# zhenfeizhang/falcon-r1cs

Hardware: AMD Instinct MI355X
Metric: falcon1024_verify_with_ntt_r1cs_witnesses_per_sec (higher is better)
Workload: dtype u32; 1 GPU; falcon-1024 full verify-with-ntt witness (NTT ladder + mod_q + pointwise + l2-norm), batch=65536 signatures per GPU per step (BASELINE configs[2] on every GPU); logn=10, batch_per_gpu=65536, chunk=32768, encoding=bls12-381-fr montgomery (arkworks witness_assignment bytes), seed=0x46414c434f4e31, signatures_failing_range_checks=0, ranks_seen=1, hbm_plan_bytes=166888865792, hbm_plan_limit_bytes=259200000000

## Files before the change

### falcon-r1cs_amd/csrc/frw_keccak.h

```cpp
#pragma once
#include <hip/hip_runtime.h>
#include <stdint.h>

namespace frw {

static __constant__ uint64_t KECCAK_RC[24] = {
    0x0000000000000001ull, 0x0000000000008082ull, 0x800000000000808aull, 0x8000000080008000ull, 0x000000000000808bull,
    0x0000000080000001ull, 0x8000000080008081ull, 0x8000000000008009ull, 0x000000000000008aull, 0x0000000000000088ull,
    0x0000000080008009ull, 0x000000008000000aull, 0x000000008000808bull, 0x800000000000008bull, 0x8000000000008089ull,
    0x8000000000008003ull, 0x8000000000008002ull, 0x8000000000000080ull, 0x000000000000800aull, 0x800000008000000aull,
    0x8000000080008081ull, 0x8000000000008080ull, 0x0000000080000001ull, 0x8000000080008008ull};

__device__ __forceinline__ uint64_t rol64(uint64_t x, int n) { return (x << n) | (x >> (64 - n)); }

__device__ __forceinline__ void keccak_f1600(uint64_t (&a)[25])
{
#pragma unroll 1
    for (int r = 0; r < 24; r++) {
        uint64_t c0 = a[0] ^ a[5] ^ a[10] ^ a[15] ^ a[20];
        uint64_t c1 = a[1] ^ a[6] ^ a[11] ^ a[16] ^ a[21];
        uint64_t c2 = a[2] ^ a[7] ^ a[12] ^ a[17] ^ a[22];
        uint64_t c3 = a[3] ^ a[8] ^ a[13] ^ a[18] ^ a[23];
        uint64_t c4 = a[4] ^ a[9] ^ a[14] ^ a[19] ^ a[24];
        const uint64_t d0 = c4 ^ rol64(c1, 1), d1 = c0 ^ rol64(c2, 1), d2 = c1 ^ rol64(c3, 1), d3 = c2 ^ rol64(c4, 1),
                       d4 = c3 ^ rol64(c0, 1);
        const uint64_t b0 = a[0] ^ d0;
        const uint64_t b10 = rol64(a[1] ^ d1, 1), b20 = rol64(a[2] ^ d2, 62), b5 = rol64(a[3] ^ d3, 28), b15 = rol64(a[4] ^ d4, 27);
        const uint64_t b16 = rol64(a[5] ^ d0, 36), b1 = rol64(a[6] ^ d1, 44), b11 = rol64(a[7] ^ d2, 6), b21 = rol64(a[8] ^ d3, 55),
                       b6 = rol64(a[9] ^ d4, 20);
        const uint64_t b7 = rol64(a[10] ^ d0, 3), b17 = rol64(a[11] ^ d1, 10), b2 = rol64(a[12] ^ d2, 43), b12 = rol64(a[13] ^ d3, 25),
                       b22 = rol64(a[14] ^ d4, 39);
        const uint64_t b23 = rol64(a[15] ^ d0, 41), b8 = rol64(a[16] ^ d1, 45), b18 = rol64(a[17] ^ d2, 15), b3 = rol64(a[18] ^ d3, 21),
                       b13 = rol64(a[19] ^ d4, 8);
        const uint64_t b14 = rol64(a[20] ^ d0, 18), b24 = rol64(a[21] ^ d1, 2), b9 = rol64(a[22] ^ d2, 61), b19 = rol64(a[23] ^ d3, 56),
                       b4 = rol64(a[24] ^ d4, 14);
        a[0] = b0 ^ (~b1 & b2) ^ KECCAK_RC[r]; a[1] = b1 ^ (~b2 & b3); a[2] = b2 ^ (~b3 & b4); a[3] = b3 ^ (~b4 & b0); a[4] = b4 ^ (~b0 & b1);
        a[5] = b5 ^ (~b6 & b7); a[6] = b6 ^ (~b7 & b8); a[7] = b7 ^ (~b8 & b9); a[8] = b8 ^ (~b9 & b5); a[9] = b9 ^ (~b5 & b6);
        a[10] = b10 ^ (~b11 & b12); a[11] = b11 ^ (~b12 & b13); a[12] = b12 ^ (~b13 & b14); a[13] = b13 ^ (~b14 & b10); a[14] = b14 ^ (~b10 & b11);
        a[15] = b15 ^ (~b16 & b17); a[16] = b16 ^ (~b17 & b18); a[17] = b17 ^ (~b18 & b19); a[18] = b18 ^ (~b19 & b15); a[19] = b19 ^ (~b15 & b16);
        a[20] = b20 ^ (~b21 & b22); a[21] = b21 ^ (~b22 & b23); a[22] = b22 ^ (~b23 & b24); a[23] = b23 ^ (~b24 & b20); a[24] = b24 ^ (~b20 & b21);
    }
}

}
```

### falcon-r1cs_amd/csrc/frw_prepare.hip

```cpp
#include <hip/hip_runtime.h>
#include <stdint.h>
#include "frw_device.h"
#include "frw_keccak.h"

namespace frw {

constexpr int SHAKE256_RATE = 136;
constexpr int NONCE_LEN = 40;

__global__ __launch_bounds__(BLOCK) void hash_to_point_kernel(int logn, size_t batch, const uint8_t *__restrict__ nonces,
                                                              const uint8_t *__restrict__ msgs,
                                                              const uint64_t *__restrict__ msg_off, uint16_t *__restrict__ hm)
{
    const size_t s = (size_t)blockIdx.x * blockDim.x + threadIdx.x;
    if (s >= batch) return;
    const int n = 1 << logn;
    const uint8_t *nonce = nonces + s * NONCE_LEN;
    const uint8_t *msg = msgs + msg_off[s];
    const uint64_t o0 = msg_off[s], o1 = msg_off[s + 1];
    const size_t total = NONCE_LEN + (size_t)(o1 >= o0 ? o1 - o0 : 0);
    uint64_t st[25];
#pragma unroll
    for (int i = 0; i < 25; i++) st[i] = 0;
    for (size_t pos = 0;; pos += SHAKE256_RATE) {
#pragma unroll
        for (int l = 0; l < SHAKE256_RATE / 8; l++) {
            uint64_t w = 0;
#pragma unroll
            for (int b = 0; b < 8; b++) {
                const size_t p = pos + (size_t)(l * 8 + b);
                uint32_t byte = 0;
                if (p < NONCE_LEN) byte = nonce[p];
                else if (p < total) byte = msg[p - NONCE_LEN];
                else if (p == total) byte = 0x1F;
                w |= (uint64_t)byte << (8 * b);
            }
            st[l] ^= w;
        }
        const bool last = total < pos + SHAKE256_RATE;
        if (last) st[16] ^= 0x8000000000000000ull;
        keccak_f1600(st);
        if (last) break;
    }
    uint16_t *out = hm + s * (size_t)n;
    int cnt = 0;
    while (cnt < n) {
#pragma unroll
        for (int w = 0; w < SHAKE256_RATE / 2; w++) {
            const uint64_t lane = st[w / 4];
            const int sh = (w % 4) * 16;
            const uint32_t v = (uint32_t)((lane >> sh) & 0xff) << 8 | (uint32_t)((lane >> (sh + 8)) & 0xff);
            if (v < 5 * Q && cnt < n) out[cnt++] = (uint16_t)(v % Q);
        }
        if (cnt < n) keccak_f1600(st);
    }
}

__global__ __launch_bounds__(BLOCK) void decode_public_keys_kernel(int logn, size_t batch, const uint8_t *__restrict__ pk_bytes,
                                                                   uint16_t *__restrict__ pk, int32_t *__restrict__ status)
{
    const int n = 1 << logn;
    const size_t pk_len = 1 + (size_t)14 * n / 8;
    const size_t idx = (size_t)blockIdx.x * blockDim.x + threadIdx.x;
    if (idx >= batch * (size_t)n) return;
    const size_t s = idx >> logn;
    const int k = (int)(idx & (size_t)(n - 1));
    const uint8_t *p = pk_bytes + s * pk_len;
    const int bit = 14 * k, off = bit & 7;
    const uint8_t *q = p + 1 + (bit >> 3);
    uint32_t acc = (uint32_t)q[0] << 16 | (uint32_t)q[1] << 8;
    if (off + 14 > 16) acc |= q[2];
    const uint32_t c = (acc >> (24 - 14 - off)) & 0x3fffu;
    pk[idx] = (uint16_t)c;
    if (c >= Q || (k == 0 && p[0] != (uint8_t)logn)) atomicMax(&status[s], ST_DECODE);
}

__global__ __launch_bounds__(BLOCK) void decode_signatures_kernel(int logn, size_t batch, const uint8_t *__restrict__ sig_bytes,
                                                                  size_t sig_len, uint16_t *__restrict__ sig,
                                                                  uint8_t *__restrict__ nonce_out, int32_t *__restrict__ status)
{
    const size_t s = (size_t)blockIdx.x * blockDim.x + threadIdx.x;
    if (s >= batch) return;
    const int n = 1 << logn;
    const uint8_t *p = sig_bytes + s * sig_len;
    uint16_t *out = sig + s * (size_t)n;
    bool ok = sig_len > 1 + NONCE_LEN && p[0] == (uint8_t)(0x30 + logn);
    if (ok && nonce_out)
        for (int i = 0; i < NONCE_LEN; i++) nonce_out[s * NONCE_LEN + i] = p[1 + i];
    const uint8_t *body = p + 1 + NONCE_LEN;
    const size_t body_len = ok ? sig_len - 1 - NONCE_LEN : 0;
    size_t v = 0;
    uint32_t acc = 0;
    int acc_len = 0;
    for (int u = 0; ok && u < n; u++) {
        if (v >= body_len) { ok = false; break; }
        acc = (acc << 8) | body[v++];
        const uint32_t b = acc >> acc_len;
        const uint32_t sign = b & 128u;
        uint32_t m = b & 127u;
        for (;;) {
            if (acc_len == 0) {
                if (v >= body_len) { ok = false; break; }
                acc = (acc << 8) | body[v++];
                acc_len = 8;
            }
            acc_len--;
            if ((acc >> acc_len) & 1u) break;
            m += 128;
            if (m > 2047) { ok = false; break; }
        }
        if (sign && m == 0) ok = false;
        if (ok) out[u] = (uint16_t)(sign ? Q - m : m);
    }
    if (ok && (acc & ((1u << acc_len) - 1u))) ok = false;
    for (; ok && v < body_len; v++)
        if (body[v]) ok = false;
    status[s] = ok ? ST_OK : ST_DECODE;
}

hipError_t launch_hash_to_point(int logn, size_t batch, const uint8_t *nonces, const uint8_t *msgs, const uint64_t *msg_off,
                                uint16_t *hm, hipStream_t st)
{
    if (batch == 0) return hipSuccess;
    hipLaunchKernelGGL(hash_to_point_kernel, dim3((unsigned)((batch + BLOCK - 1) / BLOCK)), dim3(BLOCK), 0, st, logn, batch, nonces,
                       msgs, msg_off, hm);
    return hipGetLastError();
}

hipError_t launch_decode_public_keys(int logn, size_t batch, const uint8_t *pk_bytes, uint16_t *pk, int32_t *status, hipStream_t st)
{
    if (batch == 0) return hipSuccess;
    hipError_t e = hipMemsetAsync(status, 0, batch * sizeof(int32_t), st);
    if (e != hipSuccess) return e;
    const size_t total = batch << logn;
    hipLaunchKernelGGL(decode_public_keys_kernel, dim3((unsigned)((total + BLOCK - 1) / BLOCK)), dim3(BLOCK), 0, st, logn, batch,
                       pk_bytes, pk, status);
    return hipGetLastError();
}

hipError_t launch_decode_signatures(int logn, size_t batch, const uint8_t *sig_bytes, size_t sig_len, uint16_t *sig,
                                    uint8_t *nonce_out, int32_t *status, hipStream_t st)
{
    if (batch == 0) return hipSuccess;
    hipLaunchKernelGGL(decode_signatures_kernel, dim3((unsigned)((batch + BLOCK - 1) / BLOCK)), dim3(BLOCK), 0, st, logn, batch,
                       sig_bytes, sig_len, sig, nonce_out, status);
    return hipGetLastError();
}

}
```

Baseline: 1.296 million signatures/s.

## Rewrite input-preparation kernels: paired-lane Keccak, vectorized decoders, batched stores

Hash-to-point now splits each Keccak-f1600 state across two lanes, each holding 32-bit halves and exchanging words through DPP swaps. Absorption uses 8-byte loads and output coefficients are gathered into 16-byte stores. Public-key decode uses one block per key with 8 coefficients per thread and a block-wide OR instead of a memset plus atomics. Signature decode reads 16-byte pieces through an LDS ring and decodes 8 codewords per step with clz. These changes target uncoalesced byte-wise loads and serial scalar work in the preprocessing stage, at the cost of more complex code and the risk of alignment or edge-case bugs.

Result: no change. 1.295 million signatures/s (median of 2 runs) (-0.1%).

```diff
diff --git a/falcon-r1cs_amd/csrc/frw_codec.h b/falcon-r1cs_amd/csrc/frw_codec.h
--- /dev/null
+++ b/falcon-r1cs_amd/csrc/frw_codec.h
@@ -0,0 +1,114 @@
+#pragma once
+#include <hip/hip_runtime.h>
+#include <stddef.h>
+#include <stdint.h>
+
+namespace frw {
+
+constexpr uint32_t CODEC_Q = 12289;
+constexpr int SIG_HEADER_LEN = 1 + 40;
+
+constexpr uint32_t SIG_RING_WORDS = 32;
+
+template <class Fetch, class Ring> struct SigBodyReader {
+    Fetch fetch;
+    Ring ring;
+    uint4 s0, s1;
+    uint32_t ns;
+    uint32_t rd, wr;
+    uint32_t ahead;
+    size_t piece;
+    size_t end_off;
+    size_t left;
+    uint64_t win;
+    int have;
+
+    __host__ __device__ __forceinline__ SigBodyReader(Fetch f, Ring r, unsigned body_misalign, size_t body_len)
+        : fetch(f), ring(r), ns(0), rd(1), wr(16), piece(4), end_off(body_misalign + body_len), left(body_misalign + body_len), win(0), have(0)
+    {
+        s0 = s1 = make_uint4(0, 0, 0, 0);
+        for (uint32_t k = 0; k < 4; k++)
+            if (16 * (size_t)k < end_off) put_piece(4 * k, fetch(k));
+        ahead = ring.get(0);
+        for (unsigned i = 0; i < body_misalign / 4; i++) (void)next_word();
+        win = (uint64_t)next_word() << 32;
+        have = 32 - 8 * (int)(body_misalign & 3);
+        win <<= 8 * (body_misalign & 3);
+    }
+
+    __host__ __device__ __forceinline__ void put_piece(uint32_t at, uint4 p)
+    {
+        ring.put(at % SIG_RING_WORDS, p.x);
+        ring.put((at + 1) % SIG_RING_WORDS, p.y);
+        ring.put((at + 2) % SIG_RING_WORDS, p.z);
+        ring.put((at + 3) % SIG_RING_WORDS, p.w);
+    }
+
+    __host__ __device__ __forceinline__ void boundary()
+    {
+        if (ns >= 1) { put_piece(wr, s0); wr += 4; }
+        if (ns == 2) { put_piece(wr, s1); wr += 4; }
+        const uint32_t avail = wr - rd;
+        ns = avail >= 16 ? 0u : avail >= 12 ? 1u : 2u;
+        if (ns >= 1 && 16 * piece < end_off) s0 = fetch(piece);
+        if (ns == 2 && 16 * (piece + 1) < end_off) s1 = fetch(piece + 1);
+        piece += ns;
+    }
+
+    __host__ __device__ __forceinline__ uint32_t next_word()
+    {
+        uint32_t w = __builtin_bswap32(ahead);
+        ahead = ring.get(rd % SIG_RING_WORDS);
+        rd++;
+        if (left < 4) {
+            w = left ? w & ~(0xffffffffu >> (8 * (unsigned)left)) : 0u;
+            left = 0;
+        } else {
+            left -= 4;
+        }
+        return w;
+    }
+
+    __host__ __device__ __forceinline__ bool codeword(uint32_t &coeff)
+    {
+        if (have <= 32) {
+            win |= (uint64_t)next_word() << (32 - have);
+            have += 32;
+        }
+        const uint32_t top = (uint32_t)(win >> 32);
+        const uint32_t z = (uint32_t)__builtin_clz((top << 8) | 0x8000u);
+        const uint32_t m = ((top >> 24) & 127u) + 128u * z;
+        const bool neg = (top >> 31) != 0;
+        win <<= 9 + z;
+        have -= 9 + (int)z;
+        coeff = neg ? CODEC_Q - m : m;
+        return z <= 15 && !(neg && m == 0);
+    }
+
+    __host__ __device__ __forceinline__ bool rest_is_zero()
+    {
+        uint32_t acc = (uint32_t)(win >> 32) | (uint32_t)win;
+        while (left) {
+            boundary();
+            for (int i = 0; i < 8; i++) acc |= next_word();
+        }
+        return acc == 0;
+    }
+};
+
+template <class Fetch, class Ring, class Store8>
+__host__ __device__ __forceinline__ bool sig_decode_body(Fetch f, Ring ring, unsigned body_misalign, size_t body_len, int n, Store8 store)
+{
+    SigBodyReader<Fetch, Ring> r(f, ring, body_misalign, body_len);
+    bool ok = true;
+    for (int u = 0; ok && u < n; u += 8) {
+        uint32_t c[8];
+        r.boundary();
+#pragma unroll
+        for (int j = 0; j < 8; j++) ok &= r.codeword(c[j]);
+        if (ok) store(u, c);
+    }
+    return ok && r.rest_is_zero();
+}
+
+}
diff --git a/falcon-r1cs_amd/csrc/frw_keccak.h b/falcon-r1cs_amd/csrc/frw_keccak.h
--- a/falcon-r1cs_amd/csrc/frw_keccak.h
+++ b/falcon-r1cs_amd/csrc/frw_keccak.h
@@ -42,4 +42,49 @@
     }
 }
 
+__device__ __forceinline__ uint32_t keccak_pair_swap(uint32_t x)
+{
+    return (uint32_t)__builtin_amdgcn_update_dpp(0, (int)x, 0xB1 , 0xf, 0xf, false);
 }
+
+template <int R> __device__ __forceinline__ uint32_t rol64_half(uint32_t own)
+{
+    static_assert(R >= 0 && R < 64 && R != 32, "a rotation of Keccak-f[1600]");
+    if (R == 0) return own;
+    const uint32_t other = keccak_pair_swap(own);
+    return R < 32 ? __builtin_amdgcn_alignbit(own, other, 32 - R) : __builtin_amdgcn_alignbit(other, own, 64 - R);
+}
+
+__device__ __forceinline__ void keccak_f1600_pair(uint32_t (&a)[25], uint32_t half)
+{
+#pragma unroll 1
+    for (int r = 0; r < 24; r++) {
+        const uint32_t c0 = a[0] ^ a[5] ^ a[10] ^ a[15] ^ a[20];
+        const uint32_t c1 = a[1] ^ a[6] ^ a[11] ^ a[16] ^ a[21];
+        const uint32_t c2 = a[2] ^ a[7] ^ a[12] ^ a[17] ^ a[22];
+        const uint32_t c3 = a[3] ^ a[8] ^ a[13] ^ a[18] ^ a[23];
+        const uint32_t c4 = a[4] ^ a[9] ^ a[14] ^ a[19] ^ a[24];
+        const uint32_t d0 = c4 ^ rol64_half<1>(c1), d1 = c0 ^ rol64_half<1>(c2), d2 = c1 ^ rol64_half<1>(c3), d3 = c2 ^ rol64_half<1>(c4),
+                       d4 = c3 ^ rol64_half<1>(c0);
+        const uint32_t b0 = a[0] ^ d0;
+        const uint32_t b10 = rol64_half<1>(a[1] ^ d1), b20 = rol64_half<62>(a[2] ^ d2), b5 = rol64_half<28>(a[3] ^ d3),
+                       b15 = rol64_half<27>(a[4] ^ d4);
+        const uint32_t b16 = rol64_half<36>(a[5] ^ d0), b1 = rol64_half<44>(a[6] ^ d1), b11 = rol64_half<6>(a[7] ^ d2),
+                       b21 = rol64_half<55>(a[8] ^ d3), b6 = rol64_half<20>(a[9] ^ d4);
+        const uint32_t b7 = rol64_half<3>(a[10] ^ d0), b17 = rol64_half<10>(a[11] ^ d1), b2 = rol64_half<43>(a[12] ^ d2),
+                       b12 = rol64_half<25>(a[13] ^ d3), b22 = rol64_half<39>(a[14] ^ d4);
+        const uint32_t b23 = rol64_half<41>(a[15] ^ d0), b8 = rol64_half<45>(a[16] ^ d1), b18 = rol64_half<15>(a[17] ^ d2),
+                       b3 = rol64_half<21>(a[18] ^ d3), b13 = rol64_half<8>(a[19] ^ d4);
+        const uint32_t b14 = rol64_half<18>(a[20] ^ d0), b24 = rol64_half<2>(a[21] ^ d1), b9 = rol64_half<61>(a[22] ^ d2),
+                       b19 = rol64_half<56>(a[23] ^ d3), b4 = rol64_half<14>(a[24] ^ d4);
+        const uint64_t rc = KECCAK_RC[r];
+        a[0] = b0 ^ (~b1 & b2) ^ (half ? (uint32_t)(rc >> 32) : (uint32_t)rc);
+        a[1] = b1 ^ (~b2 & b3); a[2] = b2 ^ (~b3 & b4); a[3] = b3 ^ (~b4 & b0); a[4] = b4 ^ (~b0 & b1);
+        a[5] = b5 ^ (~b6 & b7); a[6] = b6 ^ (~b7 & b8); a[7] = b7 ^ (~b8 & b9); a[8] = b8 ^ (~b9 & b5); a[9] = b9 ^ (~b5 & b6);
+        a[10] = b10 ^ (~b11 & b12); a[11] = b11 ^ (~b12 & b13); a[12] = b12 ^ (~b13 & b14); a[13] = b13 ^ (~b14 & b10); a[14] = b14 ^ (~b10 & b11);
+        a[15] = b15 ^ (~b16 & b17); a[16] = b16 ^ (~b17 & b18); a[17] = b17 ^ (~b18 & b19); a[18] = b18 ^ (~b19 & b15); a[19] = b19 ^ (~b15 & b16);
+        a[20] = b20 ^ (~b21 & b22); a[21] = b21 ^ (~b22 & b23); a[22] = b22 ^ (~b23 & b24); a[23] = b23 ^ (~b24 & b20); a[24] = b24 ^ (~b20 & b21);
+    }
+}
+
+}
diff --git a/falcon-r1cs_amd/csrc/frw_prepare.hip b/falcon-r1cs_amd/csrc/frw_prepare.hip
--- a/falcon-r1cs_amd/csrc/frw_prepare.hip
+++ b/falcon-r1cs_amd/csrc/frw_prepare.hip
@@ -1,5 +1,6 @@
 #include <hip/hip_runtime.h>
 #include <stdint.h>
+#include "frw_codec.h"
 #include "frw_device.h"
 #include "frw_keccak.h"
 
@@ -7,134 +8,196 @@
 
 constexpr int SHAKE256_RATE = 136;
 constexpr int NONCE_LEN = 40;
-
+static_assert(CODEC_Q == Q && SIG_HEADER_LEN == 1 + NONCE_LEN, "frw_codec.h restates the constants of this unit");
+
+template <bool ALIGNED> __device__ __forceinline__ void store8(uint16_t *dst, uint32_t c0, uint32_t c1, uint32_t c2, uint32_t c3,
+                                                               uint32_t c4, uint32_t c5, uint32_t c6, uint32_t c7)
+{
+    if (ALIGNED) {
+        *reinterpret_cast<uint4 *>(dst) = make_uint4(c0 | c1 << 16, c2 | c3 << 16, c4 | c5 << 16, c6 | c7 << 16);
+    } else {
+        dst[0] = (uint16_t)c0; dst[1] = (uint16_t)c1; dst[2] = (uint16_t)c2; dst[3] = (uint16_t)c3;
+        dst[4] = (uint16_t)c4; dst[5] = (uint16_t)c5; dst[6] = (uint16_t)c6; dst[7] = (uint16_t)c7;
+    }
+}
+
+__device__ __forceinline__ uint64_t load8(const uint8_t *p)
+{
+    const uintptr_t a = reinterpret_cast<uintptr_t>(p);
+    const uint64_t *q = reinterpret_cast<const uint64_t *>(a & ~(uintptr_t)7);
+    const unsigned sh = 8u * (unsigned)(a & 7);
+    uint64_t w = q[0];
+    if (sh) w = (w >> sh) | (q[1] << (64 - sh));
+    return w;
+}
+
+template <bool ALIGNED>
 __global__ __launch_bounds__(BLOCK) void hash_to_point_kernel(int logn, size_t batch, const uint8_t *__restrict__ nonces,
                                                               const uint8_t *__restrict__ msgs,
                                                               const uint64_t *__restrict__ msg_off, uint16_t *__restrict__ hm)
 {
-    const size_t s = (size_t)blockIdx.x * blockDim.x + threadIdx.x;
+    const size_t t = (size_t)blockIdx.x * blockDim.x + threadIdx.x;
+    const size_t s = t >> 1;
+    const uint32_t half = (uint32_t)(t & 1);
     if (s >= batch) return;
-    const int n = 1 << logn;
+    const uint32_t n = 1u << logn;
     const uint8_t *nonce = nonces + s * NONCE_LEN;
     const uint8_t *msg = msgs + msg_off[s];
     const uint64_t o0 = msg_off[s], o1 = msg_off[s + 1];
-    const size_t total = NONCE_LEN + (size_t)(o1 >= o0 ? o1 - o0 : 0);
-    uint64_t st[25];
+    const size_t mlen = (size_t)(o1 >= o0 ? o1 - o0 : 0);
+    const size_t total = NONCE_LEN + mlen;
+    uint32_t st[25];
 #pragma unroll
     for (int i = 0; i < 25; i++) st[i] = 0;
     for (size_t pos = 0;; pos += SHAKE256_RATE) {
 #pragma unroll
         for (int l = 0; l < SHAKE256_RATE / 8; l++) {
+            const size_t p = pos + (size_t)(l * 8);
             uint64_t w = 0;
-#pragma unroll
-            for (int b = 0; b < 8; b++) {
-                const size_t p = pos + (size_t)(l * 8 + b);
-                uint32_t byte = 0;
-                if (p < NONCE_LEN) byte = nonce[p];
-                else if (p < total) byte = msg[p - NONCE_LEN];
-                else if (p == total) byte = 0x1F;
-                w |= (uint64_t)byte << (8 * b);
+            if (p + 8 <= NONCE_LEN) {
+                w = load8(nonce + p);
+            } else if (p + 8 <= total) {
+                w = load8(msg + (p - NONCE_LEN));
+            } else if (p <= total) {
+                for (size_t b = p; b < total; b++) w |= (uint64_t)msg[b - NONCE_LEN] << (8 * (b - p));
+                w |= (uint64_t)0x1F << (8 * (total - p));
             }
-            st[l] ^= w;
+            st[l] ^= half ? (uint32_t)(w >> 32) : (uint32_t)w;
         }
         const bool last = total < pos + SHAKE256_RATE;
-        if (last) st[16] ^= 0x8000000000000000ull;
-        keccak_f1600(st);
+        if (last && half) st[16] ^= 0x80000000u;
+        keccak_f1600_pair(st, half);
         if (last) break;
     }
     uint16_t *out = hm + s * (size_t)n;
-    int cnt = 0;
-    while (cnt < n) {
-#pragma unroll
-        for (int w = 0; w < SHAKE256_RATE / 2; w++) {
-            const uint64_t lane = st[w / 4];
-            const int sh = (w % 4) * 16;
-            const uint32_t v = (uint32_t)((lane >> sh) & 0xff) << 8 | (uint32_t)((lane >> (sh + 8)) & 0xff);
-            if (v < 5 * Q && cnt < n) out[cnt++] = (uint16_t)(v % Q);
+    uint32_t cnt = 0;
+    uint32_t g0 = 0, g1 = 0, g2 = 0, g3 = 0;
+    for (;;) {
+        uint32_t hi[SHAKE256_RATE / 8];
+#pragma unroll
+        for (int l = 0; l < SHAKE256_RATE / 8; l++) hi[l] = keccak_pair_swap(st[l]);
+        if (half == 0) {
+#pragma unroll
+            for (int w = 0; w < SHAKE256_RATE / 2; w++) {
+                const uint32_t word = (w % 4 / 2) ? hi[w / 4] : st[w / 4];
+                const uint32_t le = (w % 2) ? word >> 16 : word & 0xffffu;
+                const uint32_t v = (le & 0xffu) << 8 | le >> 8;
+                if (v < 5 * Q && cnt < n) {
+                    g0 = g0 >> 16 | g1 << 16;
+                    g1 = g1 >> 16 | g2 << 16;
+                    g2 = g2 >> 16 | g3 << 16;
+                    g3 = g3 >> 16 | (v % Q) << 16;
+                    cnt++;
+                    if ((cnt & 7u) == 0)
+                        store8<ALIGNED>(out + cnt - 8, g0 & 0xffffu, g0 >> 16, g1 & 0xffffu, g1 >> 16, g2 & 0xffffu, g2 >> 16,
+                                        g3 & 0xffffu, g3 >> 16);
+                }
+            }
         }
-        if (cnt < n) keccak_f1600(st);
-    }
-}
-
-__global__ __launch_bounds__(BLOCK) void decode_public_keys_kernel(int logn, size_t batch, const uint8_t *__restrict__ pk_bytes,
-                                                                   uint16_t *__restrict__ pk, int32_t *__restrict__ status)
-{
-    const int n = 1 << logn;
-    const size_t pk_len = 1 + (size_t)14 * n / 8;
-    const size_t idx = (size_t)blockIdx.x * blockDim.x + threadIdx.x;
-    if (idx >= batch * (size_t)n) return;
-    const size_t s = idx >> logn;
-    const int k = (int)(idx & (size_t)(n - 1));
+        const uint32_t partner_cnt = keccak_pair_swap(cnt);
+        if (half) cnt = partner_cnt;
+        if (cnt >= n) break;
+        keccak_f1600_pair(st, half);
+    }
+}
+
+template <bool ALIGNED>
+__global__ __launch_bounds__(128) void decode_public_keys_kernel(int logn, size_t batch, const uint8_t *__restrict__ pk_bytes,
+                                                                 uint16_t *__restrict__ pk, int32_t *__restrict__ status)
+{
+    const size_t n = (size_t)1 << logn;
+    const size_t pk_len = 1 + 14 * n / 8;
+    const size_t s = blockIdx.x;
+    const unsigned t = threadIdx.x;
     const uint8_t *p = pk_bytes + s * pk_len;
-    const int bit = 14 * k, off = bit & 7;
-    const uint8_t *q = p + 1 + (bit >> 3);
-    uint32_t acc = (uint32_t)q[0] << 16 | (uint32_t)q[1] << 8;
-    if (off + 14 > 16) acc |= q[2];
-    const uint32_t c = (acc >> (24 - 14 - off)) & 0x3fffu;
-    pk[idx] = (uint16_t)c;
-    if (c >= Q || (k == 0 && p[0] != (uint8_t)logn)) atomicMax(&status[s], ST_DECODE);
-}
-
-__global__ __launch_bounds__(BLOCK) void decode_signatures_kernel(int logn, size_t batch, const uint8_t *__restrict__ sig_bytes,
-                                                                  size_t sig_len, uint16_t *__restrict__ sig,
-                                                                  uint8_t *__restrict__ nonce_out, int32_t *__restrict__ status)
-{
+    const uintptr_t a = reinterpret_cast<uintptr_t>(p + 1 + 14 * (size_t)t);
+    const uintptr_t end = reinterpret_cast<uintptr_t>(pk_bytes + batch * pk_len);
+    const uint32_t *q = reinterpret_cast<const uint32_t *>(a & ~(uintptr_t)3);
+    const unsigned sh = 8u * (unsigned)(a & 3);
+    uint32_t w[5];
+#pragma unroll
+    for (int i = 0; i < 5; i++) w[i] = (i < 4 || reinterpret_cast<uintptr_t>(q + i) < end) ? q[i] : 0u;
+    uint32_t be[4];
+#pragma unroll
+    for (int i = 0; i < 4; i++) be[i] = __builtin_bswap32((uint32_t)((((uint64_t)w[i + 1] << 32) | w[i]) >> sh));
+    uint32_t c[8];
+    bool bad = t == 0 && p[0] != (uint8_t)logn;
+#pragma unroll
+    for (int i = 0; i < 8; i++) {
+        const int j = 14 * i / 32, r = 14 * i % 32;
+        const uint64_t two = (uint64_t)be[j] << 32 | (j + 1 < 4 ? be[j + 1] : 0u);
+        c[i] = (uint32_t)(two >> (64 - 14 - r)) & 0x3fffu;
+        bad |= c[i] >= Q;
+    }
+    store8<ALIGNED>(pk + s * n + 8 * (size_t)t, c[0], c[1], c[2], c[3], c[4], c[5], c[6], c[7]);
+    const int any = __syncthreads_or(bad);
+    if (t == 0) status[s] = any ? ST_DECODE : ST_OK;
+}
+
+struct SigPieceFetch {
+    const uint4 *base;
+    __device__ __forceinline__ uint4 operator()(size_t k) const { return base[k]; }
+};
+struct SigLaneRing {
+    uint32_t *col;
+    __device__ __forceinline__ uint32_t get(uint32_t i) const { return col[i * WAVE]; }
+    __device__ __forceinline__ void put(uint32_t i, uint32_t w) const { col[i * WAVE] = w; }
+};
+template <bool ALIGNED> struct SigGroupStore {
+    uint16_t *row;
+    __device__ __forceinline__ void operator()(int u, const uint32_t (&c)[8]) const
+    {
+        store8<ALIGNED>(row + u, c[0], c[1], c[2], c[3], c[4], c[5], c[6], c[7]);
+    }
+};
+
+template <bool ALIGNED>
+__global__ __launch_bounds__(WAVE) void decode_signatures_kernel(int logn, size_t batch, const uint8_t *__restrict__ sig_bytes,
+                                                                 size_t sig_len, uint16_t *__restrict__ sig,
+                                                                 uint8_t *__restrict__ nonce_out, int32_t *__restrict__ status)
+{
+    __shared__ uint32_t ring[SIG_RING_WORDS][WAVE];
     const size_t s = (size_t)blockIdx.x * blockDim.x + threadIdx.x;
     if (s >= batch) return;
     const int n = 1 << logn;
     const uint8_t *p = sig_bytes + s * sig_len;
     uint16_t *out = sig + s * (size_t)n;
-    bool ok = sig_len > 1 + NONCE_LEN && p[0] == (uint8_t)(0x30 + logn);
-    if (ok && nonce_out)
-        for (int i = 0; i < NONCE_LEN; i++) nonce_out[s * NONCE_LEN + i] = p[1 + i];
-    const uint8_t *body = p + 1 + NONCE_LEN;
-    const size_t body_len = ok ? sig_len - 1 - NONCE_LEN : 0;
-    size_t v = 0;
-    uint32_t acc = 0;
-    int acc_len = 0;
-    for (int u = 0; ok && u < n; u++) {
-        if (v >= body_len) { ok = false; break; }
-        acc = (acc << 8) | body[v++];
-        const uint32_t b = acc >> acc_len;
-        const uint32_t sign = b & 128u;
-        uint32_t m = b & 127u;
-        for (;;) {
-            if (acc_len == 0) {
-                if (v >= body_len) { ok = false; break; }
-                acc = (acc << 8) | body[v++];
-                acc_len = 8;
-            }
-            acc_len--;
-            if ((acc >> acc_len) & 1u) break;
-            m += 128;
-            if (m > 2047) { ok = false; break; }
+    bool ok = sig_len > SIG_HEADER_LEN && p[0] == (uint8_t)(0x30 + logn);
+    if (ok && nonce_out) {
+        uint8_t *no = nonce_out + s * NONCE_LEN;
+        if ((reinterpret_cast<uintptr_t>(nonce_out) & 7) == 0) {
+#pragma unroll
+            for (int i = 0; i < NONCE_LEN / 8; i++) reinterpret_cast<uint64_t *>(no)[i] = load8(p + 1 + 8 * i);
+        } else {
+            for (int i = 0; i < NONCE_LEN; i++) no[i] = p[1 + i];
         }
-        if (sign && m == 0) ok = false;
-        if (ok) out[u] = (uint16_t)(sign ? Q - m : m);
-    }
-    if (ok && (acc & ((1u << acc_len) - 1u))) ok = false;
-    for (; ok && v < body_len; v++)
-        if (body[v]) ok = false;
+    }
+    if (ok) {
+        const uintptr_t body = reinterpret_cast<uintptr_t>(p + SIG_HEADER_LEN);
+        ok = sig_decode_body(SigPieceFetch{reinterpret_cast<const uint4 *>(body & ~(uintptr_t)15)}, SigLaneRing{&ring[0][threadIdx.x]},
+                             (unsigned)(body & 15), sig_len - SIG_HEADER_LEN, n, SigGroupStore<ALIGNED>{out});
+    }
+    if (!ok)
+        for (int u = 0; u < n; u += 8) store8<ALIGNED>(out + u, 0, 0, 0, 0, 0, 0, 0, 0);
     status[s] = ok ? ST_OK : ST_DECODE;
 }
+
+static bool aligned16(const void *p) { return (reinterpret_cast<uintptr_t>(p) & 15) == 0; }
 
 hipError_t launch_hash_to_point(int logn, size_t batch, const uint8_t *nonces, const uint8_t *msgs, const uint64_t *msg_off,
                                 uint16_t *hm, hipStream_t st)
 {
     if (batch == 0) return hipSuccess;
-    hipLaunchKernelGGL(hash_to_point_kernel, dim3((unsigned)((batch + BLOCK - 1) / BLOCK)), dim3(BLOCK), 0, st, logn, batch, nonces,
-                       msgs, msg_off, hm);
+    hipLaunchKernelGGL(aligned16(hm) ? hash_to_point_kernel<true> : hash_to_point_kernel<false>,
+                       dim3((unsigned)((2 * batch + BLOCK - 1) / BLOCK)), dim3(BLOCK), 0, st, logn, batch, nonces, msgs, msg_off, hm);
     return hipGetLastError();
 }
 
 hipError_t launch_decode_public_keys(int logn, size_t batch, const uint8_t *pk_bytes, uint16_t *pk, int32_t *status, hipStream_t st)
 {
     if (batch == 0) return hipSuccess;
-    hipError_t e = hipMemsetAsync(status, 0, batch * sizeof(int32_t), st);
-    if (e != hipSuccess) return e;
-    const size_t total = batch << logn;
-    hipLaunchKernelGGL(decode_public_keys_kernel, dim3((unsigned)((total + BLOCK - 1) / BLOCK)), dim3(BLOCK), 0, st, logn, batch,
-                       pk_bytes, pk, status);
+    hipLaunchKernelGGL(aligned16(pk) ? decode_public_keys_kernel<true> : decode_public_keys_kernel<false>, dim3((unsigned)batch),
+                       dim3(1u << (logn - 3)), 0, st, logn, batch, pk_bytes, pk, status);
     return hipGetLastError();
 }
 
@@ -142,8 +205,9 @@
                                     uint8_t *nonce_out, int32_t *status, hipStream_t st)
 {
     if (batch == 0) return hipSuccess;
-    hipLaunchKernelGGL(decode_signatures_kernel, dim3((unsigned)((batch + BLOCK - 1) / BLOCK)), dim3(BLOCK), 0, st, logn, batch,
-                       sig_bytes, sig_len, sig, nonce_out, status);
+    hipLaunchKernelGGL(aligned16(sig) ? decode_signatures_kernel<true> : decode_signatures_kernel<false>,
+                       dim3((unsigned)((batch + WAVE - 1) / WAVE)), dim3(WAVE), 0, st, logn, batch, sig_bytes, sig_len, sig, nonce_out,
+                       status);
     return hipGetLastError();
 }
 
```
